# lean-dojo/ReProver

Hardware: NVIDIA H100
Metric: premises encoded/sec (reindex_corpus, ByT5-small, seq_len<=512) (higher is better)
Workload: dtype bf16

## Files before the change

### reprover_b200/csrc/rpx_gemm_launch.cuh

```cuda
#pragma once
#include "rpx_common.cuh"
#include "rpx_gemm.cuh"
#include "rpx_gemm_ws.cuh"

namespace rpx {

constexpr int kGemmStages = 4;

template <int BLOCK_N, class Epi, bool M_FASTEST = false, int STAGES = kGemmStages, bool SPLIT_B = false, int BM = kBlockM>
int launch_gemm(const void* A, int64_t lda, const void* B, int64_t ldb, int M, int N, int K,
                const typename Epi::Params& ep, cudaStream_t stream, int grid_limit = 0, const void* prefetch_ptr = nullptr,
                size_t prefetch_bytes = 0) {
  using Cfg = GemmCfg<BLOCK_N, STAGES, BM>;
  static_assert(BM == kBlockM || (!M_FASTEST && Epi::kWarps == 4), "64-row tiles: encoder epilogues with one warp per lane group");
  RPX_REQUIRE(M > 0 && N > 0 && K > 0, RPX_ERR_INVALID, "gemm: empty problem M=%d N=%d K=%d", M, N, K);
  RPX_REQUIRE(K % kBlockK == 0, RPX_ERR_UNSUPPORTED, "gemm: K=%d must be a multiple of %d", K, kBlockK);
  RPX_REQUIRE(M_FASTEST || N % 32 == 0, RPX_ERR_UNSUPPORTED, "gemm: N=%d must be a multiple of 32", N);
  DeviceInfo dev;
  RPX_TRY(get_device_info(&dev));
  CUtensorMap tmA, tmB;
  RPX_TRY(make_tmap_bf16_2d(&tmA, A, (uint64_t)M, (uint64_t)K, (uint64_t)lda, BM));
  RPX_TRY(make_tmap_bf16_2d(&tmB, B, (uint64_t)N, (uint64_t)K, (uint64_t)ldb, SPLIT_B ? BLOCK_N / 2 : BLOCK_N));
  RPX_REQUIRE(!SPLIT_B || N % BLOCK_N == 0, RPX_ERR_UNSUPPORTED, "gemm: split-B tiles need N %% %d == 0", BLOCK_N);
  const int tiles_m = ceil_div(M, BM);
  const int tiles_n = ceil_div(N, BLOCK_N);
  const size_t smem = Cfg::smem_bytes(Epi::kSmemBytes);
  RPX_REQUIRE(smem <= dev.smem_optin, RPX_ERR_UNSUPPORTED, "gemm: needs %zu B smem, device allows %zu",
              smem, dev.smem_optin);
  auto kern = gemm_tc_kernel<BLOCK_N, STAGES, Epi, M_FASTEST, SPLIT_B, BM>;
  static thread_local int configured_dev = -1;
  if (configured_dev != dev.device) {
    RPX_CUDA_OK(cudaFuncSetAttribute(kern, cudaFuncAttributeMaxDynamicSharedMemorySize, (int)smem));
    configured_dev = dev.device;
  }
  int grid = tiles_m * tiles_n;
  int cap = grid_limit > 0 ? grid_limit : dev.num_sms;
  if (grid > cap) grid = cap;
  L2Prefetch pf{prefetch_ptr, (uint32_t)prefetch_bytes, grid, next_timeline_slot()};
  if (prefetch_ptr != nullptr && prefetch_bytes > 0 && prefetch_bytes < ((size_t)1 << 32) && grid < dev.num_sms)
    grid = dev.num_sms;
  RPX_CUDA_OK(launch_pdl(kern, dim3(grid), dim3(gemm_threads<Epi>()), smem, stream, pdl_enabled(), tmA, tmB, M, N, K, tiles_m,
                         tiles_n, 1, ep, pf));
  return RPX_OK;
}

constexpr int kFfnUpStages = 4;
constexpr int kFfnUpCluster = 2;

template <class Epi, int STAGES, int CLUSTER>
int launch_gemm_ws(const void* A, int64_t lda, const void* B, int64_t ldb, int M, int N, int K,
                   const typename Epi::Params& ep, cudaStream_t stream) {
  RPX_REQUIRE(M > 0 && N > 0 && K > 0, RPX_ERR_INVALID, "gemm: empty problem M=%d N=%d K=%d", M, N, K);
  RPX_REQUIRE(K % kBlockK == 0, RPX_ERR_UNSUPPORTED, "gemm: K=%d must be a multiple of %d", K, kBlockK);
  RPX_REQUIRE(N % 32 == 0, RPX_ERR_UNSUPPORTED, "gemm: N=%d must be a multiple of 32", N);
  DeviceInfo dev;
  RPX_TRY(get_device_info(&dev));
  CUtensorMap tmA, tmB, tmR;
  RPX_TRY(make_tmap_bf16_2d(&tmA, A, (uint64_t)M, (uint64_t)K, (uint64_t)lda, kBlockM));
  RPX_TRY(make_tmap_bf16_2d(&tmB, B, (uint64_t)N, (uint64_t)K, (uint64_t)ldb, kWsBlockN / CLUSTER));
  if constexpr (Epi::kResBufs > 0)
    RPX_TRY(make_tmap_2d(&tmR, 4, ep.h32, (uint64_t)M, (uint64_t)N, (uint64_t)ep.ld, kResChunkCols, 64, 128));
  else
    tmR = tmA;
  const int tiles_m = ceil_div(M, kBlockM);
  const int tiles_n = ceil_div(N, kWsBlockN);
  const size_t smem = WsCfg<STAGES, Epi::kResBufs>::kSmemBytes;
  RPX_REQUIRE(smem <= dev.smem_optin, RPX_ERR_UNSUPPORTED, "gemm: needs %zu B smem, device allows %zu", smem,
              dev.smem_optin);
  auto kern = gemm_ws_kernel<Epi, STAGES, CLUSTER>;
  static thread_local int configured_dev = -1;
  static thread_local int max_clusters = 0;
  if (configured_dev != dev.device) {
    RPX_CUDA_OK(cudaFuncSetAttribute(kern, cudaFuncAttributeMaxDynamicSharedMemorySize, (int)smem));
    cudaLaunchConfig_t cfg{};
    cfg.gridDim = dim3(CLUSTER * dev.num_sms);
    cfg.blockDim = dim3(kWsThreads);
    cfg.dynamicSmemBytes = smem;
    cudaLaunchAttribute at[1];
    at[0].id = cudaLaunchAttributeClusterDimension;
    at[0].val.clusterDim.x = CLUSTER;
    at[0].val.clusterDim.y = 1;
    at[0].val.clusterDim.z = 1;
    cfg.attrs = at;
    cfg.numAttrs = 1;
    RPX_CUDA_OK(cudaOccupancyMaxActiveClusters(&max_clusters, kern, &cfg));
    RPX_REQUIRE(max_clusters > 0, RPX_ERR_UNSUPPORTED, "gemm: no cluster of %d CTAs with %zu B smem fits the device",
                CLUSTER, smem);
    configured_dev = dev.device;
  }
  int clusters = ceil_div(tiles_m, CLUSTER) * tiles_n;
  if (clusters > max_clusters) clusters = max_clusters;
  RPX_CUDA_OK(launch_pdl<CLUSTER>(kern, dim3(CLUSTER * clusters), dim3(kWsThreads), smem, stream, pdl_enabled(), tmA,
                                  tmB, tmR, M, N, K, tiles_m, tiles_n, ep));
  return RPX_OK;
}

template <class Epi, int STAGES = kGemmStages>
int launch_gemm_pair(const void* A, int64_t lda, const void* B, int64_t ldb, int M, int N, int K,
                     const typename Epi::Params& ep, cudaStream_t stream) {
  constexpr int BLOCK_N = 128;
  using Cfg = GemmCfg<BLOCK_N, STAGES, kBlockM>;
  RPX_REQUIRE(M > 0 && N > 0 && K > 0, RPX_ERR_INVALID, "gemm: empty problem M=%d N=%d K=%d", M, N, K);
  RPX_REQUIRE(K % kBlockK == 0, RPX_ERR_UNSUPPORTED, "gemm: K=%d must be a multiple of %d", K, kBlockK);
  RPX_REQUIRE(N % 32 == 0, RPX_ERR_UNSUPPORTED, "gemm: N=%d must be a multiple of 32", N);
  DeviceInfo dev;
  RPX_TRY(get_device_info(&dev));
  CUtensorMap tmA, tmB;
  RPX_TRY(make_tmap_bf16_2d(&tmA, A, (uint64_t)M, (uint64_t)K, (uint64_t)lda, kBlockM));
  RPX_TRY(make_tmap_bf16_2d(&tmB, B, (uint64_t)N, (uint64_t)K, (uint64_t)ldb, BLOCK_N / 2));
  const int tiles_m = ceil_div(M, kBlockM);
  const int tiles_n = ceil_div(N, BLOCK_N);
  const size_t smem = Cfg::smem_bytes(Epi::kSmemBytes);
  RPX_REQUIRE(smem <= dev.smem_optin, RPX_ERR_UNSUPPORTED, "gemm: needs %zu B smem, device allows %zu", smem,
              dev.smem_optin);
  auto kern = gemm_tc_kernel<BLOCK_N, STAGES, Epi, false, false, kBlockM, true>;
  static thread_local int configured_dev = -1;
  if (configured_dev != dev.device) {
    RPX_CUDA_OK(cudaFuncSetAttribute(kern, cudaFuncAttributeMaxDynamicSharedMemorySize, (int)smem));
    configured_dev = dev.device;
  }
  int pairs = ceil_div(tiles_m, 2) * tiles_n;
  if (pairs > dev.num_sms / 2) pairs = dev.num_sms / 2;
  cudaLaunchConfig_t cfg{};
  cfg.gridDim = dim3(2 * pairs);
  cfg.blockDim = dim3(gemm_threads<Epi>());
  cfg.dynamicSmemBytes = smem;
  cfg.stream = stream;
  cudaLaunchAttribute at[1];
  at[0].id = cudaLaunchAttributeClusterDimension;
  at[0].val.clusterDim.x = 2;
  at[0].val.clusterDim.y = 1;
  at[0].val.clusterDim.z = 1;
  cfg.attrs = at;
  cfg.numAttrs = 1;
  RPX_CUDA_OK(cudaLaunchKernelEx(&cfg, kern, tmA, tmB, M, N, K, tiles_m, tiles_n, 1, ep,
                                 L2Prefetch{nullptr, 0u, 2 * pairs, next_timeline_slot()}));
  return RPX_OK;
}

}
```

### reprover_b200/csrc/rpx_gemm_ws.cuh

```cuda
#pragma once
#include "rpx_gemm.cuh"

namespace rpx {

constexpr int kWsBlockN = 256;
constexpr int kWsThreads = 384;
constexpr int kResChunkCols = 32;
constexpr int kResChunkBytes = 64 * kResChunkCols * 4;

template <int STAGES, int RES_BUFS>
struct WsCfg {
  static_assert(2 * STAGES + 4 * RES_BUFS <= 32, "barrier block holds 32 mbarriers");
  static constexpr int kABytes = kBlockM * kBlockK * 2;
  static constexpr int kBBytes = kWsBlockN * kBlockK * 2;
  static constexpr int kStageBytes = kABytes + kBBytes;
  static constexpr int kRingBytes = STAGES * kStageBytes;
  static constexpr int kResBytes = 2 * RES_BUFS * kResChunkBytes;
  static constexpr size_t kSmemBytes = (size_t)kRingBytes + kResBytes + 1024 + 256;
};

struct FragCtx {
  int m0, n0;
  int n_blk;
  int n_cols;
  int M, N;
  int r0;
  int q;
};

struct ResStream {
  float* buf;
  uint64_t* full;
  uint64_t* empty;
};

template <class Epi, int STAGES, int CLUSTER>
__global__ void __launch_bounds__(kWsThreads, 1)
gemm_ws_kernel(const __grid_constant__ CUtensorMap tmA, const __grid_constant__ CUtensorMap tmB,
               const __grid_constant__ CUtensorMap tmR, int M, int N, int K, int tiles_m, int tiles_n,
               typename Epi::Params ep) {
  static_assert(CLUSTER == 1 || CLUSTER == 2, "one CTA, or a pair sharing the B tile");
  using Cfg = WsCfg<STAGES, Epi::kResBufs>;
  constexpr int R = Epi::kResBufs;
  extern __shared__ uint8_t smem_raw[];
  const uint32_t raw_addr = smem_u32(smem_raw);
  uint8_t* smem = smem_raw + ((1024 - (raw_addr & 1023)) & 1023);
  uint8_t* sA = smem;
  uint8_t* sB = smem + STAGES * Cfg::kABytes;
  float* sR = reinterpret_cast<float*>(smem + Cfg::kRingBytes);
  uint64_t* full = reinterpret_cast<uint64_t*>(smem + Cfg::kRingBytes + Cfg::kResBytes);
  uint64_t* empty = full + STAGES;
  uint64_t* rfull = empty + STAGES;
  uint64_t* rempty = rfull + 2 * R;

  const int warp = threadIdx.x >> 5;
  const int wg = warp >> 2;
  const int num_kb = K / kBlockK;
  const int rank = CLUSTER > 1 ? (int)cluster_ctarank() : 0;
  const int num_units = (tiles_m + CLUSTER - 1) / CLUSTER * tiles_n;
  const int u0 = (int)blockIdx.x / CLUSTER;
  const int u_step = (int)gridDim.x / CLUSTER;
  auto unit_m = [&](int u) { return CLUSTER * (u / tiles_n) + rank; };

  if (threadIdx.x == 0) {
    tma_prefetch_desc(&tmA);
    tma_prefetch_desc(&tmB);
    if (R > 0) tma_prefetch_desc(&tmR);
    for (int s = 0; s < STAGES; ++s) {
      mbar_init(&full[s], 1);
      mbar_init(&empty[s], CLUSTER * 8);
    }
    for (int s = 0; s < 2 * R; ++s) {
      mbar_init(&rfull[s], 1);
      mbar_init(&rempty[s], 128);
    }
    fence_mbar_init();
  }
  __syncthreads();
  if (CLUSTER > 1) cluster_sync_all();
  pdl_launch_dependents();
  pdl_wait();

  if (wg == 0) {
    setmaxnreg_dec<40>();
    if (warp == 0 && elect_one()) {
      int stage = 0;
      uint32_t phase = 0;
      for (int u = u0; u < num_units; u += u_step) {
        const int m_blk = unit_m(u), n_blk = u % tiles_n;
        for (int kb = 0; kb < num_kb; ++kb) {
          mbar_wait(&empty[stage], phase ^ 1);
          mbar_arrive_expect_tx(&full[stage], Cfg::kStageBytes);
          tma_load_2d(sA + stage * Cfg::kABytes, &tmA, &full[stage], kb * kBlockK, m_blk * kBlockM);
          if constexpr (CLUSTER == 1) {
            tma_load_2d(sB + stage * Cfg::kBBytes, &tmB, &full[stage], kb * kBlockK, n_blk * kWsBlockN);
          } else {
            constexpr int H = kWsBlockN / 2;
            tma_load_2d_multicast(sB + stage * Cfg::kBBytes + rank * H * kBlockK * 2, &tmB, &full[stage], kb * kBlockK,
                                  n_blk * kWsBlockN + rank * H, (uint16_t)0x3);
          }
          if (++stage == STAGES) {
            stage = 0;
            phase ^= 1;
          }
        }
      }
    } else if (R > 0 && (warp == 1 || warp == 2) && elect_one()) {
      const int w = warp - 1;
      float* buf = sR + w * R * (kResChunkBytes / 4);
      uint64_t* rf = rfull + w * R;
      uint64_t* re = rempty + w * R;
      int b = 0;
      uint32_t phase = 0;
      for (int u = u0; u < num_units; u += u_step) {
        const int row0 = unit_m(u) * kBlockM + 64 * w;
        const int n0 = (u % tiles_n) * kWsBlockN;
        const int n_cols = N - n0 < kWsBlockN ? N - n0 : kWsBlockN;
        if (row0 >= M) continue;
        for (int col = 0; col < n_cols; col += kResChunkCols) {
          mbar_wait(&re[b], phase ^ 1);
          mbar_arrive_expect_tx(&rf[b], kResChunkBytes);
          tma_load_2d(buf + b * (kResChunkBytes / 4), &tmR, &rf[b], n0 + col, row0);
          if (++b == R) {
            b = 0;
            phase ^= 1;
          }
        }
      }
    }
  } else {
    setmaxnreg_inc<232>();
    const int cw = wg - 1;
    const int lane = threadIdx.x & 31;
    Epi epi(ep, ResStream{sR + cw * R * (kResChunkBytes / 4), rfull + cw * R, rempty + cw * R});
    float acc[128];
    int stage = 0;
    uint32_t phase = 0;
    auto release = [&](int st) {
      __syncwarp();
      if (lane == 0) {
        mbar_arrive(&empty[st]);
        if (CLUSTER > 1) mbar_arrive_cluster(&empty[st], (uint32_t)(rank ^ 1));
      }
    };
    for (int u = u0; u < num_units; u += u_step) {
      FragCtx c;
      c.n_blk = u % tiles_n;
      c.m0 = unit_m(u) * kBlockM;
      c.n0 = c.n_blk * kWsBlockN;
      c.n_cols = N - c.n0 < kWsBlockN ? N - c.n0 : kWsBlockN;
      c.M = M;
      c.N = N;
      c.r0 = c.m0 + 64 * cw + 16 * (warp & 3) + (lane >> 2);
      c.q = lane & 3;
      int prev = 0;
      for (int kb = 0; kb < num_kb; ++kb) {
        mbar_wait(&full[stage], phase);
        const uint64_t a_desc = make_smem_desc_kmajor_sw128(smem_u32(sA + stage * Cfg::kABytes)) + 512 * cw;
        const uint64_t b_desc = make_smem_desc_kmajor_sw128(smem_u32(sB + stage * Cfg::kBBytes));
        wgmma_fence_operand(acc);
        wgmma_fence();
#pragma unroll
        for (int k = 0; k < kBlockK / kMmaK; ++k) wgmma_m64n256k16_ss(acc, a_desc + 2 * k, b_desc + 2 * k, (kb | k) != 0);
        wgmma_commit();
        if (kb == 0) epi.prefetch(c);
        if (kb > 0) {
          wgmma_wait<1>();
          release(prev);
        }
        prev = stage;
        if (++stage == STAGES) {
          stage = 0;
          phase ^= 1;
        }
      }
      wgmma_wait<0>();
      wgmma_fence_operand(acc);
      release(prev);
      epi.tile(c, acc);
    }
  }
  if (CLUSTER > 1) {
    __syncwarp();
    cluster_sync_all();
  }
}


struct EpiWsStoreF32 {
  using Params = EpiStoreF32::Params;
  static constexpr int kResBufs = 0;
  Params p;
  __device__ EpiWsStoreF32(const Params& p_, const ResStream&) : p(p_) {}
  __device__ void prefetch(const FragCtx&) {}
  __device__ void tile(const FragCtx& c, const float (&acc)[128]) {
#pragma unroll
    for (int j = 0; j < 32; ++j) {
      if (8 * j < c.n_cols) {
        float* dst = p.C + (size_t)c.r0 * p.ldc + c.n0 + 8 * j + 2 * c.q;
        if (c.r0 < c.M) *reinterpret_cast<float2*>(dst) = make_float2(acc[4 * j], acc[4 * j + 1]);
        if (c.r0 + 8 < c.M) *reinterpret_cast<float2*>(dst + 8 * (size_t)p.ldc) = make_float2(acc[4 * j + 2], acc[4 * j + 3]);
      }
    }
  }
};

struct EpiWsGeGLU {
  struct Params {
    __nv_bfloat16* out;
    int ldo;
    RowScale rs;
  };
  static constexpr int kResBufs = 0;
  Params p;
  float rs0 = 0.f, rs1 = 0.f;
  __device__ EpiWsGeGLU(const Params& p_, const ResStream&) : p(p_) {}
  __device__ void prefetch(const FragCtx& c) {
    rs0 = c.r0 < c.M ? p.rs.get(c.r0) : 0.f;
    rs1 = c.r0 + 8 < c.M ? p.rs.get(c.r0 + 8) : 0.f;
  }
  __device__ void tile(const FragCtx& c, const float (&acc)[128]) {
    __nv_bfloat16* dst = p.out + (size_t)c.r0 * p.ldo + c.n_blk * (kWsBlockN / 2) + 2 * c.q;
#pragma unroll
    for (int j = 0; j < 16; ++j) {
      const float* g = acc + 4 * j;
      const float* u = acc + 4 * (j + 16);
      if (c.r0 < c.M)
        *reinterpret_cast<uint32_t*>(dst + 8 * j) =
            pack_bf16x2(gelu_new(g[0] * rs0) * (u[0] * rs0), gelu_new(g[1] * rs0) * (u[1] * rs0));
      if (c.r0 + 8 < c.M)
        *reinterpret_cast<uint32_t*>(dst + 8 * (size_t)p.ldo + 8 * j) =
            pack_bf16x2(gelu_new(g[2] * rs1) * (u[2] * rs1), gelu_new(g[3] * rs1) * (u[3] * rs1));
    }
  }
};

template <int RES_BUFS>
struct EpiWsResidual {
  using Params = EpiResidualParams;
  static constexpr int kResBufs = RES_BUFS;
  Params p;
  ResStream rs;
  int b = 0;
  uint32_t phase = 0;
  __device__ EpiWsResidual(const Params& p_, const ResStream& rs_) : p(p_), rs(rs_) {}
  __device__ void prefetch(const FragCtx&) {}
  __device__ void tile(const FragCtx& c, const float (&acc)[128]) {
    const int lane = threadIdx.x & 31;
    const int v = (threadIdx.x >> 5) & 3;
    const int row0 = c.r0 - 16 * v - (lane >> 2);
    if (row0 >= c.M) return;
    const int sub = lane >> 3, j4 = lane & 7;
    float ss[4];
#pragma unroll
    for (int k = 0; k < kWsBlockN / kResChunkCols; ++k) {
      if (kResChunkCols * k >= c.n_cols) break;
      if (k % 4 == 0) {
#pragma unroll
        for (int i = 0; i < 4; ++i) ss[i] = 0.f;
      }
      float* s = rs.buf + b * (kResChunkBytes / 4);
      mbar_wait(&rs.full[b], phase);
#pragma unroll
      for (int jj = 0; jj < 4; ++jj) {
        const int j = 4 * k + jj;
#pragma unroll
        for (int h = 0; h < 2; ++h) {
          const int r = 16 * v + (lane >> 2) + 8 * h;
          float2* x = reinterpret_cast<float2*>(s + r * kResChunkCols + (((2 * jj + (c.q >> 1)) ^ (r & 7)) << 2) + 2 * (c.q & 1));
          float2 hv = *x;
          hv.x += acc[4 * j + 2 * h];
          hv.y += acc[4 * j + 2 * h + 1];
          *x = hv;
        }
      }
      __syncwarp();
      const size_t col = (size_t)c.n0 + kResChunkCols * k + 4 * j4;
#pragma unroll
      for (int i = 0; i < 4; ++i) {
        const int r = 16 * v + sub + 4 * i;
        const int m = row0 + r;
        const float4 hv = *reinterpret_cast<const float4*>(s + r * kResChunkCols + ((j4 ^ (r & 7)) << 2));
        ss[i] += hv.x * hv.x + hv.y * hv.y + hv.z * hv.z + hv.w * hv.w;
        if (m < c.M) {
          *reinterpret_cast<float4*>(p.h32 + (size_t)m * p.ld + col) = hv;
          *reinterpret_cast<uint2*>(p.h16 + (size_t)m * p.ld + col) =
              make_uint2(pack_bf16x2(hv.x, hv.y), pack_bf16x2(hv.z, hv.w));
        }
      }
      fence_proxy_async_smem();
      mbar_arrive(&rs.empty[b]);
      if (++b == RES_BUFS) {
        b = 0;
        phase ^= 1;
      }
      if (k % 4 == 3 || kResChunkCols * (k + 1) >= c.n_cols) {
        const int part = 2 * c.n_blk + k / 4;
#pragma unroll
        for (int i = 0; i < 4; ++i) {
          float t = ss[i];
          t += __shfl_xor_sync(0xffffffffu, t, 1);
          t += __shfl_xor_sync(0xffffffffu, t, 2);
          t += __shfl_xor_sync(0xffffffffu, t, 4);
          const int m = row0 + 16 * v + sub + 4 * i;
          if (j4 == 0 && m < c.M) p.ss_out[(size_t)part * p.ss_stride + m] = t;
        }
      }
    }
  }
};

}
```

### reprover_b200/csrc/rpx_ptx.cuh

```cuda
#pragma once
#include <cuda_runtime.h>
#include <cuda_bf16.h>
#include <stdint.h>

namespace rpx {

#define RPX_DEVICE __device__ __forceinline__

RPX_DEVICE uint32_t smem_u32(const void* p) {
  return static_cast<uint32_t>(__cvta_generic_to_shared(p));
}

RPX_DEVICE uint32_t lane_id() { return threadIdx.x & 31; }

RPX_DEVICE uint32_t elect_one() {
  uint32_t pred = 0;
  asm volatile(
      "{\n"
      ".reg .b32 rx;\n"
      ".reg .pred px;\n"
      "elect.sync rx|px, 0xFFFFFFFF;\n"
      "@px mov.s32 %0, 1;\n"
      "}\n"
      : "+r"(pred));
  return pred;
}

RPX_DEVICE void mbar_init(uint64_t* bar, uint32_t count) {
  asm volatile("mbarrier.init.shared::cta.b64 [%0], %1;" ::"r"(smem_u32(bar)), "r"(count));
}
RPX_DEVICE void fence_mbar_init() {
  asm volatile("fence.mbarrier_init.release.cluster;" ::: "memory");
}
RPX_DEVICE void fence_proxy_async_smem() {
  asm volatile("fence.proxy.async.shared::cta;" ::: "memory");
}
RPX_DEVICE void mbar_arrive_expect_tx(uint64_t* bar, uint32_t bytes) {
  asm volatile("mbarrier.arrive.expect_tx.shared::cta.b64 _, [%0], %1;" ::"r"(smem_u32(bar)),
               "r"(bytes)
               : "memory");
}
RPX_DEVICE void mbar_arrive(uint64_t* bar) {
  asm volatile("mbarrier.arrive.shared::cta.b64 _, [%0];" ::"r"(smem_u32(bar)) : "memory");
}
#ifndef RPX_WAIT_HINT_NS
#define RPX_WAIT_HINT_NS 2000
#endif
template <uint32_t HINT_NS>
RPX_DEVICE uint32_t mbar_try_wait_t(uint64_t* bar, uint32_t parity) {
  uint32_t ok;
  if constexpr (HINT_NS > 0) {
    asm volatile(
        "{\n"
        ".reg .pred p;\n"
        "mbarrier.try_wait.parity.shared::cta.b64 p, [%1], %2, %3;\n"
        "selp.u32 %0, 1, 0, p;\n"
        "}\n"
        : "=r"(ok)
        : "r"(smem_u32(bar)), "r"(parity), "r"(HINT_NS)
        : "memory");
  } else {
    asm volatile(
        "{\n"
        ".reg .pred p;\n"
        "mbarrier.try_wait.parity.shared::cta.b64 p, [%1], %2;\n"
        "selp.u32 %0, 1, 0, p;\n"
        "}\n"
        : "=r"(ok)
        : "r"(smem_u32(bar)), "r"(parity)
        : "memory");
  }
  return ok;
}
template <uint32_t HINT_NS = RPX_WAIT_HINT_NS>
RPX_DEVICE void mbar_wait(uint64_t* bar, uint32_t parity) {
  if (mbar_try_wait_t<HINT_NS>(bar, parity)) return;
  uint32_t spins = 0;
  long long t0 = 0;
  while (!mbar_try_wait_t<HINT_NS>(bar, parity)) {
    if ((++spins & 0x3FFu) == 0) {
      const long long now = clock64();
      if (t0 == 0) t0 = now;
      if (now - t0 > 4000000000LL) __trap();
    }
  }
}

RPX_DEVICE void tma_load_2d(void* smem_dst, const void* tmap, uint64_t* bar, int32_t c0,
                            int32_t c1) {
  asm volatile(
      "cp.async.bulk.tensor.2d.shared::cluster.global.mbarrier::complete_tx::bytes"
      " [%0], [%1, {%3, %4}], [%2];"
      :
      : "r"(smem_u32(smem_dst)), "l"(reinterpret_cast<uint64_t>(tmap)), "r"(smem_u32(bar)),
        "r"(c0), "r"(c1)
      : "memory");
}
RPX_DEVICE void tma_load_2d_hint(void* smem_dst, const void* tmap, uint64_t* bar, int32_t c0,
                                 int32_t c1, uint64_t policy) {
  asm volatile(
      "cp.async.bulk.tensor.2d.shared::cluster.global.mbarrier::complete_tx::bytes.L2::cache_hint"
      " [%0], [%1, {%3, %4}], [%2], %5;"
      :
      : "r"(smem_u32(smem_dst)), "l"(reinterpret_cast<uint64_t>(tmap)), "r"(smem_u32(bar)),
        "r"(c0), "r"(c1), "l"(policy)
      : "memory");
}
RPX_DEVICE void tma_load_2d_multicast(void* smem_dst, const void* tmap, uint64_t* bar, int32_t c0, int32_t c1,
                                      uint16_t cta_mask) {
  asm volatile(
      "cp.async.bulk.tensor.2d.shared::cluster.global.mbarrier::complete_tx::bytes.multicast::cluster"
      " [%0], [%1, {%3, %4}], [%2], %5;"
      :
      : "r"(smem_u32(smem_dst)), "l"(reinterpret_cast<uint64_t>(tmap)), "r"(smem_u32(bar)), "r"(c0), "r"(c1),
        "h"(cta_mask)
      : "memory");
}
RPX_DEVICE void tma_store_2d(const void* tmap, const void* smem_src, int32_t c0, int32_t c1) {
  asm volatile("cp.async.bulk.tensor.2d.global.shared::cta.bulk_group [%0, {%2, %3}], [%1];" ::"l"(
                   reinterpret_cast<uint64_t>(tmap)),
               "r"(smem_u32(smem_src)), "r"(c0), "r"(c1)
               : "memory");
}
RPX_DEVICE void bulk_commit_group() { asm volatile("cp.async.bulk.commit_group;" ::: "memory"); }
template <int N>
RPX_DEVICE void bulk_wait_group_read() {
  asm volatile("cp.async.bulk.wait_group.read %0;" ::"n"(N) : "memory");
}
constexpr uint64_t kEvictFirst = 0x12F0000000000000ull;
constexpr uint64_t kEvictLast = 0x14F0000000000000ull;
constexpr uint64_t kEvictNormal = 0x1000000000000000ull;

RPX_DEVICE void tma_prefetch_desc(const void* tmap) {
  asm volatile("prefetch.tensormap [%0];" ::"l"(reinterpret_cast<uint64_t>(tmap)) : "memory");
}

RPX_DEVICE uint32_t cluster_ctarank() {
  uint32_t r;
  asm volatile("mov.u32 %0, %%cluster_ctarank;" : "=r"(r));
  return r;
}
RPX_DEVICE void cluster_sync_all() {
  asm volatile("barrier.cluster.arrive.release.aligned;" ::: "memory");
  asm volatile("barrier.cluster.wait.acquire.aligned;" ::: "memory");
}
RPX_DEVICE void mbar_arrive_cluster(uint64_t* bar, uint32_t cta) {
  asm volatile(
      "{\n"
      ".reg .b32 ra;\n"
      "mapa.shared::cluster.u32 ra, %0, %1;\n"
      "mbarrier.arrive.shared::cluster.b64 _, [ra];\n"
      "}\n" ::"r"(smem_u32(bar)),
      "r"(cta)
      : "memory");
}

RPX_DEVICE void wgmma_fence() { asm volatile("wgmma.fence.sync.aligned;" ::: "memory"); }
RPX_DEVICE void wgmma_commit() { asm volatile("wgmma.commit_group.sync.aligned;" ::: "memory"); }
template <int N>
RPX_DEVICE void wgmma_wait() {
  asm volatile("wgmma.wait_group.sync.aligned %0;" ::"n"(N) : "memory");
}
template <int R>
RPX_DEVICE void wgmma_fence_operand(float (&d)[R]) {
#pragma unroll
  for (int i = 0; i < R; ++i) asm volatile("" : "+f"(d[i])::"memory");
}

RPX_DEVICE void wgmma_m64n64k16_ss(float (&d)[32], uint64_t desc_a, uint64_t desc_b, uint32_t accumulate) {
  asm volatile(
      "{\n"
      ".reg .pred p;\n"
      "setp.ne.b32 p, %34, 0;\n"
      "wgmma.mma_async.sync.aligned.m64n64k16.f32.bf16.bf16 "
      "{%0, %1, %2, %3, %4, %5, %6, %7, %8, %9, %10, %11, %12, %13, %14, %15, %16, %17, %18, %19, %20, %21, %22, %23, %24, %25, %26, %27, %28, %29, %30, %31}, %32, %33, p, 1, 1, 0, 0;\n"
      "}\n"
      : "+f"(d[0]), "+f"(d[1]), "+f"(d[2]), "+f"(d[3]), "+f"(d[4]), "+f"(d[5]), "+f"(d[6]), "+f"(d[7]), "+f"(d[8]), "+f"(d[9]), "+f"(d[10]), "+f"(d[11]), "+f"(d[12]), "+f"(d[13]), "+f"(d[14]), "+f"(d[15]), "+f"(d[16]), "+f"(d[17]), "+f"(d[18]), "+f"(d[19]), "+f"(d[20]), "+f"(d[21]), "+f"(d[22]), "+f"(d[23]), "+f"(d[24]), "+f"(d[25]), "+f"(d[26]), "+f"(d[27]), "+f"(d[28]), "+f"(d[29]), "+f"(d[30]), "+f"(d[31])
      : "l"(desc_a), "l"(desc_b), "r"(accumulate));
}

RPX_DEVICE void wgmma_m64n128k16_ss(float (&d)[64], uint64_t desc_a, uint64_t desc_b, uint32_t accumulate) {
  asm volatile(
      "{\n"
      ".reg .pred p;\n"
      "setp.ne.b32 p, %66, 0;\n"
      "wgmma.mma_async.sync.aligned.m64n128k16.f32.bf16.bf16 "
      "{%0, %1, %2, %3, %4, %5, %6, %7, %8, %9, %10, %11, %12, %13, %14, %15, %16, %17, %18, %19, %20, %21, %22, %23, %24, %25, %26, %27, %28, %29, %30, %31, %32, %33, %34, %35, %36, %37, %38, %39, %40, %41, %42, %43, %44, %45, %46, %47, %48, %49, %50, %51, %52, %53, %54, %55, %56, %57, %58, %59, %60, %61, %62, %63}, %64, %65, p, 1, 1, 0, 0;\n"
      "}\n"
      : "+f"(d[0]), "+f"(d[1]), "+f"(d[2]), "+f"(d[3]), "+f"(d[4]), "+f"(d[5]), "+f"(d[6]), "+f"(d[7]), "+f"(d[8]), "+f"(d[9]), "+f"(d[10]), "+f"(d[11]), "+f"(d[12]), "+f"(d[13]), "+f"(d[14]), "+f"(d[15]), "+f"(d[16]), "+f"(d[17]), "+f"(d[18]), "+f"(d[19]), "+f"(d[20]), "+f"(d[21]), "+f"(d[22]), "+f"(d[23]), "+f"(d[24]), "+f"(d[25]), "+f"(d[26]), "+f"(d[27]), "+f"(d[28]), "+f"(d[29]), "+f"(d[30]), "+f"(d[31]), "+f"(d[32]), "+f"(d[33]), "+f"(d[34]), "+f"(d[35]), "+f"(d[36]), "+f"(d[37]), "+f"(d[38]), "+f"(d[39]), "+f"(d[40]), "+f"(d[41]), "+f"(d[42]), "+f"(d[43]), "+f"(d[44]), "+f"(d[45]), "+f"(d[46]), "+f"(d[47]), "+f"(d[48]), "+f"(d[49]), "+f"(d[50]), "+f"(d[51]), "+f"(d[52]), "+f"(d[53]), "+f"(d[54]), "+f"(d[55]), "+f"(d[56]), "+f"(d[57]), "+f"(d[58]), "+f"(d[59]), "+f"(d[60]), "+f"(d[61]), "+f"(d[62]), "+f"(d[63])
      : "l"(desc_a), "l"(desc_b), "r"(accumulate));
}

RPX_DEVICE void wgmma_m64n256k16_ss(float (&d)[128], uint64_t desc_a, uint64_t desc_b, uint32_t accumulate) {
  asm volatile(
      "{\n"
      ".reg .pred p;\n"
      "setp.ne.b32 p, %130, 0;\n"
      "wgmma.mma_async.sync.aligned.m64n256k16.f32.bf16.bf16 "
      "{%0, %1, %2, %3, %4, %5, %6, %7, %8, %9, %10, %11, %12, %13, %14, %15, %16, %17, %18, %19, %20, %21, %22, %23, %24, %25, %26, %27, %28, %29, %30, %31, %32, %33, %34, %35, %36, %37, %38, %39, %40, %41, %42, %43, %44, %45, %46, %47, %48, %49, %50, %51, %52, %53, %54, %55, %56, %57, %58, %59, %60, %61, %62, %63, %64, %65, %66, %67, %68, %69, %70, %71, %72, %73, %74, %75, %76, %77, %78, %79, %80, %81, %82, %83, %84, %85, %86, %87, %88, %89, %90, %91, %92, %93, %94, %95, %96, %97, %98, %99, %100, %101, %102, %103, %104, %105, %106, %107, %108, %109, %110, %111, %112, %113, %114, %115, %116, %117, %118, %119, %120, %121, %122, %123, %124, %125, %126, %127}, %128, %129, p, 1, 1, 0, 0;\n"
      "}\n"
      : "+f"(d[0]), "+f"(d[1]), "+f"(d[2]), "+f"(d[3]), "+f"(d[4]), "+f"(d[5]), "+f"(d[6]), "+f"(d[7]), "+f"(d[8]), "+f"(d[9]), "+f"(d[10]), "+f"(d[11]), "+f"(d[12]), "+f"(d[13]), "+f"(d[14]), "+f"(d[15]), "+f"(d[16]), "+f"(d[17]), "+f"(d[18]), "+f"(d[19]), "+f"(d[20]), "+f"(d[21]), "+f"(d[22]), "+f"(d[23]), "+f"(d[24]), "+f"(d[25]), "+f"(d[26]), "+f"(d[27]), "+f"(d[28]), "+f"(d[29]), "+f"(d[30]), "+f"(d[31]), "+f"(d[32]), "+f"(d[33]), "+f"(d[34]), "+f"(d[35]), "+f"(d[36]), "+f"(d[37]), "+f"(d[38]), "+f"(d[39]), "+f"(d[40]), "+f"(d[41]), "+f"(d[42]), "+f"(d[43]), "+f"(d[44]), "+f"(d[45]), "+f"(d[46]), "+f"(d[47]), "+f"(d[48]), "+f"(d[49]), "+f"(d[50]), "+f"(d[51]), "+f"(d[52]), "+f"(d[53]), "+f"(d[54]), "+f"(d[55]), "+f"(d[56]), "+f"(d[57]), "+f"(d[58]), "+f"(d[59]), "+f"(d[60]), "+f"(d[61]), "+f"(d[62]), "+f"(d[63]), "+f"(d[64]), "+f"(d[65]), "+f"(d[66]), "+f"(d[67]), "+f"(d[68]), "+f"(d[69]), "+f"(d[70]), "+f"(d[71]), "+f"(d[72]), "+f"(d[73]), "+f"(d[74]), "+f"(d[75]), "+f"(d[76]), "+f"(d[77]), "+f"(d[78]), "+f"(d[79]), "+f"(d[80]), "+f"(d[81]), "+f"(d[82]), "+f"(d[83]), "+f"(d[84]), "+f"(d[85]), "+f"(d[86]), "+f"(d[87]), "+f"(d[88]), "+f"(d[89]), "+f"(d[90]), "+f"(d[91]), "+f"(d[92]), "+f"(d[93]), "+f"(d[94]), "+f"(d[95]), "+f"(d[96]), "+f"(d[97]), "+f"(d[98]), "+f"(d[99]), "+f"(d[100]), "+f"(d[101]), "+f"(d[102]), "+f"(d[103]), "+f"(d[104]), "+f"(d[105]), "+f"(d[106]), "+f"(d[107]), "+f"(d[108]), "+f"(d[109]), "+f"(d[110]), "+f"(d[111]), "+f"(d[112]), "+f"(d[113]), "+f"(d[114]), "+f"(d[115]), "+f"(d[116]), "+f"(d[117]), "+f"(d[118]), "+f"(d[119]), "+f"(d[120]), "+f"(d[121]), "+f"(d[122]), "+f"(d[123]), "+f"(d[124]), "+f"(d[125]), "+f"(d[126]), "+f"(d[127])
      : "l"(desc_a), "l"(desc_b), "r"(accumulate));
}

RPX_DEVICE void wgmma_m64n64k16_rs_bmn(float (&d)[32], const uint32_t (&a)[4], uint64_t desc_b, uint32_t accumulate) {
  asm volatile(
      "{\n"
      ".reg .pred p;\n"
      "setp.ne.b32 p, %37, 0;\n"
      "wgmma.mma_async.sync.aligned.m64n64k16.f32.bf16.bf16 "
      "{%0, %1, %2, %3, %4, %5, %6, %7, %8, %9, %10, %11, %12, %13, %14, %15, %16, %17, %18, %19, %20, %21, %22, %23, %24, %25, %26, %27, %28, %29, %30, %31}, {%32, %33, %34, %35}, %36, p, 1, 1, 1;\n"
      "}\n"
      : "+f"(d[0]), "+f"(d[1]), "+f"(d[2]), "+f"(d[3]), "+f"(d[4]), "+f"(d[5]), "+f"(d[6]), "+f"(d[7]), "+f"(d[8]), "+f"(d[9]), "+f"(d[10]), "+f"(d[11]), "+f"(d[12]), "+f"(d[13]), "+f"(d[14]), "+f"(d[15]), "+f"(d[16]), "+f"(d[17]), "+f"(d[18]), "+f"(d[19]), "+f"(d[20]), "+f"(d[21]), "+f"(d[22]), "+f"(d[23]), "+f"(d[24]), "+f"(d[25]), "+f"(d[26]), "+f"(d[27]), "+f"(d[28]), "+f"(d[29]), "+f"(d[30]), "+f"(d[31])
      : "r"(a[0]), "r"(a[1]), "r"(a[2]), "r"(a[3]), "l"(desc_b), "r"(accumulate));
}

RPX_DEVICE uint64_t make_smem_desc_sw128(uint32_t smem_addr, uint32_t lbo_bytes) {
  uint64_t d = 0;
  d |= static_cast<uint64_t>((smem_addr & 0x3FFFF) >> 4);
  d |= static_cast<uint64_t>(lbo_bytes >> 4) << 16;
  d |= static_cast<uint64_t>(1024 >> 4) << 32;
  d |= static_cast<uint64_t>(1) << 62;
  return d;
}
RPX_DEVICE uint64_t make_smem_desc_kmajor_sw128(uint32_t smem_addr) { return make_smem_desc_sw128(smem_addr, 16); }
RPX_DEVICE uint64_t make_smem_desc_mnmajor_sw128(uint32_t smem_addr) { return make_smem_desc_sw128(smem_addr, 1024); }

RPX_DEVICE void pdl_wait() { asm volatile("griddepcontrol.wait;" ::: "memory"); }
RPX_DEVICE void pdl_launch_dependents() { asm volatile("griddepcontrol.launch_dependents;" ::: "memory"); }

template <uint32_t N>
RPX_DEVICE void setmaxnreg_dec() { asm volatile("setmaxnreg.dec.sync.aligned.u32 %0;" ::"n"(N)); }
template <uint32_t N>
RPX_DEVICE void setmaxnreg_inc() { asm volatile("setmaxnreg.inc.sync.aligned.u32 %0;" ::"n"(N)); }

RPX_DEVICE uint32_t pack_bf16x2(float lo, float hi) {
  __nv_bfloat162 v = __floats2bfloat162_rn(lo, hi);
  return *reinterpret_cast<uint32_t*>(&v);
}

}
```

Measured before the change: 4377.

## Stage GeGLU epilogue output in swizzled smem and write it with TMA stores

The warp-specialized GeGLU epilogue used to write packed bf16 pairs straight to global memory from registers, one scattered 4-byte store per fragment. It now writes them into a per-consumer-warpgroup 128B-swizzled shared buffer and issues two TMA 2D stores per tile. Each tile waits for the previous bulk store to finish reading the buffer, and a drain at kernel end waits for all stores. The aim is to coalesce output traffic and take store issue off the math warps, at the cost of extra shared memory, named-barrier syncs and a new output tensor map.

```diff
diff --git a/reprover_b200/csrc/rpx_gemm_launch.cuh b/reprover_b200/csrc/rpx_gemm_launch.cuh
--- a/reprover_b200/csrc/rpx_gemm_launch.cuh
+++ b/reprover_b200/csrc/rpx_gemm_launch.cuh
@@ -60,11 +60,13 @@
   RPX_TRY(make_tmap_bf16_2d(&tmB, B, (uint64_t)N, (uint64_t)K, (uint64_t)ldb, kWsBlockN / CLUSTER));
   if constexpr (Epi::kResBufs > 0)
     RPX_TRY(make_tmap_2d(&tmR, 4, ep.h32, (uint64_t)M, (uint64_t)N, (uint64_t)ep.ld, kResChunkCols, 64, 128));
+  else if constexpr (Epi::kOutBytes > 0)
+    RPX_TRY(Epi::make_out_map(&tmR, ep, M, N));
   else
     tmR = tmA;
   const int tiles_m = ceil_div(M, kBlockM);
   const int tiles_n = ceil_div(N, kWsBlockN);
-  const size_t smem = WsCfg<STAGES, Epi::kResBufs>::kSmemBytes;
+  const size_t smem = WsCfg<STAGES, Epi::kResBufs, Epi::kOutBytes>::kSmemBytes;
   RPX_REQUIRE(smem <= dev.smem_optin, RPX_ERR_UNSUPPORTED, "gemm: needs %zu B smem, device allows %zu", smem,
               dev.smem_optin);
   auto kern = gemm_ws_kernel<Epi, STAGES, CLUSTER>;
diff --git a/reprover_b200/csrc/rpx_gemm_ws.cuh b/reprover_b200/csrc/rpx_gemm_ws.cuh
--- a/reprover_b200/csrc/rpx_gemm_ws.cuh
+++ b/reprover_b200/csrc/rpx_gemm_ws.cuh
@@ -8,15 +8,17 @@
 constexpr int kResChunkCols = 32;
 constexpr int kResChunkBytes = 64 * kResChunkCols * 4;
 
-template <int STAGES, int RES_BUFS>
+template <int STAGES, int RES_BUFS, int OUT_BYTES = 0>
 struct WsCfg {
   static_assert(2 * STAGES + 4 * RES_BUFS <= 32, "barrier block holds 32 mbarriers");
+  static_assert(OUT_BYTES % 1024 == 0, "output staging keeps the 1024-byte alignment of 128B swizzle");
   static constexpr int kABytes = kBlockM * kBlockK * 2;
   static constexpr int kBBytes = kWsBlockN * kBlockK * 2;
   static constexpr int kStageBytes = kABytes + kBBytes;
   static constexpr int kRingBytes = STAGES * kStageBytes;
   static constexpr int kResBytes = 2 * RES_BUFS * kResChunkBytes;
-  static constexpr size_t kSmemBytes = (size_t)kRingBytes + kResBytes + 1024 + 256;
+  static constexpr int kOutBytes = 2 * OUT_BYTES;
+  static constexpr size_t kSmemBytes = (size_t)kRingBytes + kResBytes + kOutBytes + 1024 + 256;
 };
 
 struct FragCtx {
@@ -34,13 +36,19 @@
   uint64_t* empty;
 };
 
+struct OutStage {
+  uint8_t* buf;
+  const CUtensorMap* tm;
+};
+
 template <class Epi, int STAGES, int CLUSTER>
 __global__ void __launch_bounds__(kWsThreads, 1)
 gemm_ws_kernel(const __grid_constant__ CUtensorMap tmA, const __grid_constant__ CUtensorMap tmB,
                const __grid_constant__ CUtensorMap tmR, int M, int N, int K, int tiles_m, int tiles_n,
                typename Epi::Params ep) {
   static_assert(CLUSTER == 1 || CLUSTER == 2, "one CTA, or a pair sharing the B tile");
-  using Cfg = WsCfg<STAGES, Epi::kResBufs>;
+  static_assert(Epi::kResBufs == 0 || Epi::kOutBytes == 0, "tmR maps either the residual or the output");
+  using Cfg = WsCfg<STAGES, Epi::kResBufs, Epi::kOutBytes>;
   constexpr int R = Epi::kResBufs;
   extern __shared__ uint8_t smem_raw[];
   const uint32_t raw_addr = smem_u32(smem_raw);
@@ -48,7 +56,8 @@
   uint8_t* sA = smem;
   uint8_t* sB = smem + STAGES * Cfg::kABytes;
   float* sR = reinterpret_cast<float*>(smem + Cfg::kRingBytes);
-  uint64_t* full = reinterpret_cast<uint64_t*>(smem + Cfg::kRingBytes + Cfg::kResBytes);
+  uint8_t* sO = smem + Cfg::kRingBytes + Cfg::kResBytes;
+  uint64_t* full = reinterpret_cast<uint64_t*>(smem + Cfg::kRingBytes + Cfg::kResBytes + Cfg::kOutBytes);
   uint64_t* empty = full + STAGES;
   uint64_t* rfull = empty + STAGES;
   uint64_t* rempty = rfull + 2 * R;
@@ -65,7 +74,7 @@
   if (threadIdx.x == 0) {
     tma_prefetch_desc(&tmA);
     tma_prefetch_desc(&tmB);
-    if (R > 0) tma_prefetch_desc(&tmR);
+    if (R > 0 || Epi::kOutBytes > 0) tma_prefetch_desc(&tmR);
     for (int s = 0; s < STAGES; ++s) {
       mbar_init(&full[s], 1);
       mbar_init(&empty[s], CLUSTER * 8);
@@ -132,7 +141,8 @@
     setmaxnreg_inc<232>();
     const int cw = wg - 1;
     const int lane = threadIdx.x & 31;
-    Epi epi(ep, ResStream{sR + cw * R * (kResChunkBytes / 4), rfull + cw * R, rempty + cw * R});
+    Epi epi(ep, ResStream{sR + cw * R * (kResChunkBytes / 4), rfull + cw * R, rempty + cw * R},
+            OutStage{sO + cw * Epi::kOutBytes, &tmR});
     float acc[128];
     int stage = 0;
     uint32_t phase = 0;
@@ -179,6 +189,7 @@
       release(prev);
       epi.tile(c, acc);
     }
+    epi.drain();
   }
   if (CLUSTER > 1) {
     __syncwarp();
@@ -190,9 +201,11 @@
 struct EpiWsStoreF32 {
   using Params = EpiStoreF32::Params;
   static constexpr int kResBufs = 0;
+  static constexpr int kOutBytes = 0;
   Params p;
-  __device__ EpiWsStoreF32(const Params& p_, const ResStream&) : p(p_) {}
+  __device__ EpiWsStoreF32(const Params& p_, const ResStream&, const OutStage&) : p(p_) {}
   __device__ void prefetch(const FragCtx&) {}
+  __device__ void drain() {}
   __device__ void tile(const FragCtx& c, const float (&acc)[128]) {
 #pragma unroll
     for (int j = 0; j < 32; ++j) {
@@ -212,26 +225,49 @@
     RowScale rs;
   };
   static constexpr int kResBufs = 0;
+  static constexpr int kOutBytes = 64 * (kWsBlockN / 2) * 2;
+  static int make_out_map(CUtensorMap* tm, const Params& p, int M, int N) {
+    return make_tmap_bf16_2d(tm, p.out, (uint64_t)M, (uint64_t)(N / 2), (uint64_t)p.ldo, 64);
+  }
   Params p;
+  OutStage os;
   float rs0 = 0.f, rs1 = 0.f;
-  __device__ EpiWsGeGLU(const Params& p_, const ResStream&) : p(p_) {}
+  __device__ EpiWsGeGLU(const Params& p_, const ResStream&, const OutStage& os_) : p(p_), os(os_) {}
   __device__ void prefetch(const FragCtx& c) {
     rs0 = c.r0 < c.M ? p.rs.get(c.r0) : 0.f;
     rs1 = c.r0 + 8 < c.M ? p.rs.get(c.r0 + 8) : 0.f;
   }
   __device__ void tile(const FragCtx& c, const float (&acc)[128]) {
-    __nv_bfloat16* dst = p.out + (size_t)c.r0 * p.ldo + c.n_blk * (kWsBlockN / 2) + 2 * c.q;
+    const int lane = threadIdx.x & 31;
+    const int v = (threadIdx.x >> 5) & 3;
+    const int row0 = c.r0 - 16 * v - (lane >> 2);
+    if (row0 >= c.M) return;
+    const bool issuer = (threadIdx.x & 127) == 0;
+    const uint32_t bar = threadIdx.x >> 7;
+    if (issuer) bulk_wait_group_read<0>();
+    bar_sync(bar, 128);
+    const int r = 16 * v + (lane >> 2);
+    const uint32_t row_addr = smem_u32(os.buf) + r * 128 + 4 * c.q;
+    const uint32_t sw = (uint32_t)(r & 7) << 4;
 #pragma unroll
     for (int j = 0; j < 16; ++j) {
       const float* g = acc + 4 * j;
       const float* u = acc + 4 * (j + 16);
-      if (c.r0 < c.M)
-        *reinterpret_cast<uint32_t*>(dst + 8 * j) =
-            pack_bf16x2(gelu_new(g[0] * rs0) * (u[0] * rs0), gelu_new(g[1] * rs0) * (u[1] * rs0));
-      if (c.r0 + 8 < c.M)
-        *reinterpret_cast<uint32_t*>(dst + 8 * (size_t)p.ldo + 8 * j) =
-            pack_bf16x2(gelu_new(g[2] * rs1) * (u[2] * rs1), gelu_new(g[3] * rs1) * (u[3] * rs1));
-    }
+      const uint32_t dst = row_addr + (j / 8) * (64 * 128) + ((uint32_t)((j % 8) << 4) ^ sw);
+      st_shared_u32(dst, pack_bf16x2(gelu_new(g[0] * rs0) * (u[0] * rs0), gelu_new(g[1] * rs0) * (u[1] * rs0)));
+      st_shared_u32(dst + 8 * 128, pack_bf16x2(gelu_new(g[2] * rs1) * (u[2] * rs1), gelu_new(g[3] * rs1) * (u[3] * rs1)));
+    }
+    fence_proxy_async_smem();
+    bar_sync(bar, 128);
+    if (issuer) {
+      const int col = c.n_blk * (kWsBlockN / 2);
+      tma_store_2d(os.tm, os.buf, col, row0);
+      tma_store_2d(os.tm, os.buf + 64 * 128, col + 64, row0);
+      bulk_commit_group();
+    }
+  }
+  __device__ void drain() {
+    if ((threadIdx.x & 127) == 0) bulk_wait_group<0>();
   }
 };
 
@@ -239,12 +275,14 @@
 struct EpiWsResidual {
   using Params = EpiResidualParams;
   static constexpr int kResBufs = RES_BUFS;
+  static constexpr int kOutBytes = 0;
   Params p;
   ResStream rs;
   int b = 0;
   uint32_t phase = 0;
-  __device__ EpiWsResidual(const Params& p_, const ResStream& rs_) : p(p_), rs(rs_) {}
+  __device__ EpiWsResidual(const Params& p_, const ResStream& rs_, const OutStage&) : p(p_), rs(rs_) {}
   __device__ void prefetch(const FragCtx&) {}
+  __device__ void drain() {}
   __device__ void tile(const FragCtx& c, const float (&acc)[128]) {
     const int lane = threadIdx.x & 31;
     const int v = (threadIdx.x >> 5) & 3;
diff --git a/reprover_b200/csrc/rpx_ptx.cuh b/reprover_b200/csrc/rpx_ptx.cuh
--- a/reprover_b200/csrc/rpx_ptx.cuh
+++ b/reprover_b200/csrc/rpx_ptx.cuh
@@ -127,6 +127,14 @@
 RPX_DEVICE void bulk_wait_group_read() {
   asm volatile("cp.async.bulk.wait_group.read %0;" ::"n"(N) : "memory");
 }
+template <int N>
+RPX_DEVICE void bulk_wait_group() {
+  asm volatile("cp.async.bulk.wait_group %0;" ::"n"(N) : "memory");
+}
+RPX_DEVICE void st_shared_u32(uint32_t addr, uint32_t v) {
+  asm volatile("st.shared.b32 [%0], %1;" ::"r"(addr), "r"(v) : "memory");
+}
+RPX_DEVICE void bar_sync(uint32_t id, uint32_t n) { asm volatile("bar.sync %0, %1;" ::"r"(id), "r"(n) : "memory"); }
 constexpr uint64_t kEvictFirst = 0x12F0000000000000ull;
 constexpr uint64_t kEvictLast = 0x14F0000000000000ull;
 constexpr uint64_t kEvictNormal = 0x1000000000000000ull;
```

Result: no change. 4400, median of 6 (+0.5%).
